# Gaukler/PlainRenderer

Measured on AMD Instinct MI355X. Metric: frames/sec full GI+shade+post @4K; %HBM roofline; 1/2/4/8-GPU scaling, higher is better.
Workload: dtype f32

## Files before the change

plainrenderer_amd/csrc/kernels_fast/shading_fast.hip:

```cpp
#include "../backend.h"
#include "../device/shading_common.h"
#include "../device/fastmath.h"
#include "../device/buffer_fetch.h"
#include "upscale_quad.h"
#include "pcf_taps.h"
#include <cstdlib>
#include <type_traits>

namespace plr {

namespace fastshade {

#ifndef PLR_SHADE_WAVES
#define PLR_SHADE_WAVES 5
#endif

PLR_DI float rcpf(float x) { return __builtin_amdgcn_rcpf(x); }
PLR_DI float rsqf(float x) { return __builtin_amdgcn_rsqf(x); }
PLR_DI float sqrtv(float x) { return __builtin_amdgcn_sqrtf(x); }
PLR_DI float fmin1(float a, float b) { return __builtin_fminf(a, b); }
PLR_DI float fmax1(float a, float b) { return __builtin_fmaxf(a, b); }
PLR_DI float fclamp(float x, float lo, float hi) { return __builtin_fminf(__builtin_fmaxf(x, lo), hi); }
PLR_DI float fmix(float a, float b, float t) { return a + (b - a) * t; }
PLR_DI float log2h(float x) { return __builtin_amdgcn_logf(x); }
// ... 21 lines not shown
    const float inv = rcpRN(sqrtRN((vx * vx + vy * vy) + vz * vz));
    o.Vn = vec3(vx * inv, vy * inv, vz * inv);
    return o;
}
struct Surface { vec3 passPos; float pixelDepth; };
PLR_DI Surface exactSurface(const GlobalUbo* __restrict__ g, vec3 Vn, float depth) {
#pragma clang fp contract(off)
    const float cx = -Vn.x, cy = -Vn.y, cz = -Vn.z;
    const float fx = g->cameraForward[0], fy = g->cameraForward[1], fz = g->cameraForward[2];
    const float dvf = (cx * fx + cy * fy) + cz * fz;
    const float den = g->farPlane + (-depth + 1.f) * (g->nearPlane - g->farPlane);
    const float depthLinear = divRN(g->nearPlane * g->farPlane, den);
    const float rd = rcpf(dvf);
    Surface s;
    s.passPos.x = g->cameraPosition[0] + divRNr(cx, dvf, rd) * depthLinear;
    s.passPos.y = g->cameraPosition[1] + divRNr(cy, dvf, rd) * depthLinear;
    s.passPos.z = g->cameraPosition[2] + divRNr(cz, dvf, rd) * depthLinear;
    const float wx = g->cameraPosition[0] - s.passPos.x, wy = g->cameraPosition[1] - s.passPos.y, wz = g->cameraPosition[2] - s.passPos.z;
    s.pixelDepth = (wx * -fx + wy * -fy) + wz * -fz;
    return s;
}

PLR_DI float D_GGX(float NoH, float r) {
    const float a = NoH * r;
    const float k = r * rcpf(1.0f - NoH * NoH + a * a);
    return k * k * (1.0f / PLR_GLSL_PI);
}
PLR_DI float Visibility(float NoV, float NoL, float r) {
    const float r_2 = r * r;
    const float v1 = NoL * sqrtv(NoV * NoV * (1.f - r_2) + r_2);
    const float v2 = NoV * sqrtv(NoL * NoL * (1.f - r_2) + r_2);
    return 0.5f * rcpf(v1 + v2);
}
PLR_DI vec3 F_Schlick(vec3 f0, vec3 f90, float VoH) { return f0 + (f90 - f0) * pow5(1.f - VoH); }
PLR_DI vec3 DisneyDiffuse(vec3 diffuseColor, float NoL, float VoH, float NoV, float r) {
    const float energyBias = 0.5f * r;
    const float energyFactor = fmix(1.f, 1.f / 1.51f, r);
    const float f90 = energyBias + 2.f * VoH * VoH * r;
    const float fl = 1.f + (f90 - 1.f) * pow5(1.f - NoL), fv = 1.f + (f90 - 1.f) * pow5(1.f - NoV);
    return diffuseColor * ((1.f / PLR_GLSL_PI) * fl * fv * energyFactor);
}
PLR_DI vec3 CoDWWIIDiffuse(vec3 diffuseColor, float NoL, float VoH, float NoV, float NoH, float r) {
    const float f0Diffuse = VoH + pow5(1.f - VoH);
    const float f1 = (1.f - 0.75f * pow5(1.f - NoL)) * (1.f - 0.75f * pow5(1.f - NoV));
    const float g = log2h(2.f * rcpf(r * r) - 1.f) * (1.f / 18.f);
    const float t = fclamp(2.2f * g - 0.5f, 0.f, 1.f);
    const float fd = f0Diffuse + (f1 - f0Diffuse) * t;
    const float fb = (34.5f * g * g - 59.f * g + 24.5f) * VoH * exp2h(-fmax1(73.2f * g - 21.2f, 8.9f) * sqrtv(NoH));
    return diffuseColor * ((1.f / PLR_GLSL_PI) * (fd + fb));
}
PLR_DI float Titanfall2DiffuseSingleComponent(float NoL, float LoV, float NoV, float NoH, float r) {
    const float facing = 0.5f + 0.5f * LoV;
    const float rough = facing * (0.9f - 0.4f * facing) * (0.5f + NoH) * rcpf(fmax1(NoH, 0.03f));
    const float smoothDiffuse = 1.05f * (1.f - pow5(1.f - NoL)) * (1.f - pow5(1.f - NoV));
    return (1.f / PLR_GLSL_PI) * fmix(smoothDiffuse, rough, r);
}
PLR_DI vec3 GGXSingleScattering(float r, vec3 f0, float NoH, float NoV, float VoH, float NoL) {
    return (D_GGX(NoH, r) * Visibility(NoV, NoL, r)) * F_Schlick(f0, vec3(1.f), VoH);
}
PLR_DI float ReflectedEnergyAverage(float roughness) {
    const float smoothness = 1.f - sqrtv(roughness);
    float r = -0.0761947f - 0.383026f * smoothness;
    r = 1.04997f + smoothness * r;
    r = 0.409255f + smoothness * r;
    return fmin1(0.999f, r);
}
PLR_DI float sRGBToLinear1(float c) {
    const float lin = c * (1.f / 12.92f), pw = fpow((c + 0.055f) * (1.f / 1.055f), 2.4f);
    return c <= 0.004045f ? lin : pw;
}

PLR_DI _Float16 halfLo(uint32_t w) { return __builtin_bit_cast(_Float16, (uint16_t)(w & 0xffffu)); }
PLR_DI _Float16 halfHi(uint32_t w) { return __builtin_bit_cast(_Float16, (uint16_t)(w >> 16)); }
PLR_DI vec4 accumulateTexel(vec4 acc, uint32_t xy, uint32_t zw, float w) {
    return vec4(__builtin_fmaf((float)halfLo(xy), w, acc.x), __builtin_fmaf((float)halfHi(xy), w, acc.y), __builtin_fmaf((float)halfLo(zw), w, acc.z),
                __builtin_fmaf((float)halfHi(zw), w, acc.w));
}
PLR_DI void edgePair(int i0, float a, int w, int* xb, float* a2) {
    *xb = clampTo(i0, w - 2);
    *a2 = __builtin_amdgcn_fmed3f(a + (float)(i0 - *xb), 0.f, 1.f);
}

PLR_DI vec4 bilinearLut(const ImgView& im, float u, float v) {
    int i0, j0; float a, b;
    linearCoord(u * (float)im.w, &i0, &a);
    linearCoord(v * (float)im.h, &j0, &b);
    int xb; float a2;
    edgePair(i0, a, im.w, &xb, &a2);
    const int y0 = clampi(j0, im.h), y1 = clampi(j0 + 1, im.h);
    const BufferDesc texels = texelBuffer(im.ptr, 8u);
    const uint4 q0 = fetch128(texels, __umul24((uint32_t)y0, (uint32_t)im.w) + (uint32_t)xb), q1 = fetch128(texels, __umul24((uint32_t)y1, (uint32_t)im.w) + (uint32_t)xb);
    const float a0 = 1.f - a2, b0 = 1.f - b;
    vec4 r(0.f);
    r = accumulateTexel(r, q0.x, q0.y, a0 * b0);
    r = accumulateTexel(r, q0.z, q0.w, a2 * b0);
    r = accumulateTexel(r, q1.x, q1.y, a0 * b);
    r = accumulateTexel(r, q1.z, q1.w, a2 * b);
    return r;
}

struct ShadeParams {
    ImgView color, depth, normal, albedo, specular, brdfLut, shadowMaps[4], ysh, cocg, volumetricLut, skyLut;
    const LightBuffer* light;
    const ShadowCascadeInfo* shadowInfo;
    const VolumetricLightingSettings* vol;
    const GlobalUbo* g;
    const ImgView* bindless;
    uint32_t bindlessCount;
    uint32_t cascadeCount;
    int coverW, coverH, yBase;
    int xBase;
    uint32_t* sig;
    ImgView noiseTex;
    const float4* pcfTaps;
    const float4* pcfTapsByPosition;
    uint32_t pcfPositions;
    const uint2* lutEnergyFootprint;
    const uint32_t* lutEnergyNonFinite;
    uint32_t skipUnlit;
};
PLR_DI float uniformValue(float x) { return u2f((uint32_t)__builtin_amdgcn_readfirstlane((int)f2u(x))); }
PLR_DI bool finiteBits(float x) { return (f2u(x) & 0x7f800000u) != 0x7f800000u; }

#define PLR_SHADE_UNIFORM_PARAMS const GlobalUbo* __restrict__ gUniform, const LightBuffer* __restrict__ lightUniform, const ShadowCascadeInfo* __restrict__ shadowUniform, \
                                 const VolumetricLightingSettings* __restrict__ volUniform
#define PLR_SHADE_ADOPT_UNIFORMS(P) do { (P).g = gUniform; (P).light = lightUniform; (P).shadowInfo = shadowUniform; (P).vol = volUniform; } while (0)
#define PLR_SHADE_UNIFORM_ARGS(P) (P).g, (P).light, (P).shadowInfo, (P).vol

struct PcfTapRow { float4 q[kPcfTaps / 2]; };
PLR_DI float calcShadow(vec3 pos, const ImgView& shadowMap, const float* __restrict__ m, float lssX, float lssY, const PcfTapRow& taps) {
    float cxy0, cxy1;
    uint32_t depthThreshold;
    {
#pragma clang fp contract(off)
        const float x = ((m[0] * pos.x + m[4] * pos.y) + m[8] * pos.z) + m[12];
        const float y = ((m[1] * pos.x + m[5] * pos.y) + m[9] * pos.z) + m[13];
        const float z = ((m[2] * pos.x + m[6] * pos.y) + m[10] * pos.z) + m[14];
        const float w = ((m[3] * pos.x + m[7] * pos.y) + m[11] * pos.z) + m[15];
        const float rw = rcpf(w);
        cxy0 = divRNr(x, w, rw) * 0.5f + 0.5f;
        cxy1 = divRNr(y, w, rw) * 0.5f + 0.5f;
        const float actualDepth = fclamp(divRNr(z, w, rw), 0.f, 1.f);
        const uint32_t t0 = (uint32_t)(actualDepth * 65535.f);
        const float r16 = 1.f / 65535.f;
        const float q1 = divRNr((float)(t0 + 1u), 65535.f, r16), q0 = divRNr((float)t0, 65535.f, r16);
        depthThreshold = q1 <= actualDepth ? t0 + 1u : (q0 <= actualDepth ? t0 : t0 - 1u);
    }
    const int w = shadowMap.w, h = shadowMap.h;
    const float fw = (float)w, fh = (float)h;
    const float bxw = fastm::clampCoord(cxy0 * fw), byh = fastm::clampCoord(cxy1 * fh);
    const float sxw = 0.03f * lssX * fw, syh = 0.03f * lssY * fh;
    const __amdgpu_buffer_rsrc_t map = __builtin_amdgcn_make_buffer_rsrc(shadowMap.ptr, 0, w * h * 2, 0x00020000);
    uint32_t lit = 0u;
// ... 1 lines not shown
        const int xi = floorToInt(__builtin_fmaf(ox, sxw, bxw)), yi = floorToInt(__builtin_fmaf(oy, syh, byh));
        const int t = __mul24(yi, w) + xi;
        const uint32_t off = (uint32_t)xi < (uint32_t)w ? (uint32_t)(t + t) : 0xffffffffu;
        const uint32_t texel = __builtin_amdgcn_raw_buffer_load_b16(map, (int)off, 0, 0);
        lit += texel <= depthThreshold ? 1u : 0u;
    };
#pragma unroll
    for (int k = 0; k < kPcfTaps / 2; k++) {
        const float4 q = taps.q[k];
        tap(q.x, q.y);
        tap(q.z, q.w);
    }
    return (float)lit * (1.f / 12.f);
}

PLR_DI float lutEnergy(const ShadeParams& P, float u, float v) {
    const ImgView& im = P.brdfLut;
    if (!P.lutEnergyFootprint) return bilinearLut(im, u, v).y;
    int i0, j0; float a, b;
    linearCoord(u * (float)im.w, &i0, &a);
    linearCoord(v * (float)im.h, &j0, &b);
    int xb, yb; float a2, b2;
    edgePair(i0, a, im.w, &xb, &a2);
    edgePair(j0, b, im.h, &yb, &b2);
    const uint2 q = P.lutEnergyFootprint[__umul24((uint32_t)yb, (uint32_t)(im.w - 1)) + (uint32_t)xb];
    const float a0 = 1.f - a2, b0 = 1.f - b2;
    float e = (float)halfLo(q.x) * (a0 * b0);
    e = __builtin_fmaf((float)halfHi(q.x), a2 * b0, e);
    e = __builtin_fmaf((float)halfLo(q.y), a0 * b2, e);
    e = __builtin_fmaf((float)halfHi(q.y), a2 * b2, e);
    return e;
}

template <int MULTISCATTER>
PLR_DI vec3 specularMultiscatteringLobe(const ShadeParams& P, float r, float NoL, vec3 f0, vec3 singleScatteringLobe, vec3 brdfLut) {
    const float energyOutgoing = brdfLut.y;
    const vec3 fresnelAverage = f0 + (1.f - f0) * (1.f / 21.f);
    if (MULTISCATTER == 0) {
        const float energyAverage = ReflectedEnergyAverage(r);
        const float energyIncoming = lutEnergy(P, r, NoL);
        const float unscaled = (1.f - energyIncoming) * (1.f - energyOutgoing) * rcpf(3.1415f * (1.f - energyAverage));
        const vec3 den = 1.f - fresnelAverage * (1.f - energyAverage);
        const vec3 scaling = (fresnelAverage * fresnelAverage * energyAverage) * vec3(rcpf(den.x), rcpf(den.y), rcpf(den.z));
        return unscaled * scaling;
    } else if (MULTISCATTER == 1) {
        const float lobe = (1.f - energyOutgoing) * (1.f / PLR_GLSL_PI);
        const vec3 den = 1.f - fresnelAverage * (1.f - energyOutgoing);
        return (fresnelAverage * fresnelAverage * (energyOutgoing * lobe)) * vec3(rcpf(den.x), rcpf(den.y), rcpf(den.z));
    } else if (MULTISCATTER == 2) {
        return f0 * (rcpf(energyOutgoing) - 1.f) * singleScatteringLobe;
    }
    return vec3(0.f);
}

struct PixelInputs {
    float depth;
    uint32_t albedo, specular;
    uint32_t normal, normalH, normalV;
    uint2 ysh;
    uint32_t cocg;
};
PLR_DI vec3 decodeNormal(uint32_t texel) {
    const vec3 raw = fastm::unorm8x4(texel).xyz() * 2.f - 1.f;
    return raw * rsqf(fmax1(dot(raw, raw), 1e-30f));
}

struct SurfaceTerms {
    vec3 N, V, f0, diffuseColor, diffuseBRDFIntegral;
    float r, NoV, energyOutgoing;
    vec3 brdfLut;
};
struct DirectOut { vec3 direct; float pixelDepth; vec2 noiseTexel; };
template <int DIFFUSE_BRDF, int MULTISCATTER, bool GEOMETRIC_AA>
PLR_DI DirectOut shadeDirect(const ShadeParams& P, bool skipUnlit, int px, int py, const ViewRay& vr, const PixelInputs& in, vec3 lightColor, SurfaceTerms* st,
                             uint32_t* sigWord) {
    constexpr bool kLobesSkippable = DIFFUSE_BRDF != 3 && (MULTISCATTER == 0 || MULTISCATTER == 3);
    uint32_t lutNonFinite = 1u;
    if (kLobesSkippable && MULTISCATTER == 0 && skipUnlit && P.lutEnergyNonFinite) lutNonFinite = *P.lutEnergyNonFinite;
    const GlobalUbo* g = P.g;
    const Surface surf = exactSurface(g, vr.Vn, in.depth);
    const vec3 passPos = surf.passPos;
    const float pixelDepth = surf.pixelDepth;

    const vec3 albedoTexel = fastm::unorm8x4(in.albedo).xyz();
    const vec3 specularTexel = fastm::unorm8x4(in.specular).xyz();
    const float metalic = specularTexel.z;
    float r = specularTexel.y;
    r = fmax1(r * r, 0.0045f);
    const vec3 albedo(sRGBToLinear1(albedoTexel.x), sRGBToLinear1(albedoTexel.y), sRGBToLinear1(albedoTexel.z));
    const vec3 diffuseColor = (1.f - metalic) * albedo;
    const vec3 N = decodeNormal(in.normal);
    const vec3 L = nrm(ld3(g->sunDirection));
    const vec3 Lu(uniformValue(L.x), uniformValue(L.y), uniformValue(L.z));
    const vec3 V = vr.Vn;
    if (GEOMETRIC_AA) {
        const vec3 N_U = decodeNormal(in.normalH) - N, N_V = decodeNormal(in.normalV) - N;
        const float variance = 0.25f * (dot(N_V, N_V) + dot(N_U, N_U));
        const float kernelRoughness2 = fmin1(2.f * variance, 0.18f);
        r = fclamp(sqrtv(r * r + kernelRoughness2), 0.f, 1.f);
    }
    const float NdotL = dot(N, L);
    const float NoL = fclamp(NdotL, 0.f, 1.f);
    const bool backFacing = NdotL <= 0.f;
    const float NoV = fmax1(fabsf(dot(N, V)), 0.0001f);
    const vec3 f0 = vmix(vec3(0.04f), albedo, metalic);

    const ImgView noiseTex = P.noiseTex;
    const uint32_t noiseIndex = fastm::texelIndex((uint32_t)fastm::repeatIndex(px, noiseTex.w), (uint32_t)fastm::repeatIndex(py, noiseTex.h), (uint32_t)noiseTex.w);
    const uint32_t noiseWord = fetch16(texelBuffer(noiseTex.ptr, 2u), noiseIndex);
    const vec2 noiseTexel = fastm::unorm8x2(noiseWord);
    const uint32_t noiseByte = noiseWord & 0xffu;

    int cascadeIndex = 0;
#pragma unroll
    for (int cascade = 0; cascade < 3; cascade++) cascadeIndex += (cascade < (int)P.cascadeCount - 1 && pixelDepth >= P.shadowInfo->splits[cascade]) ? 1 : 0;
    const bool skipLobes = kLobesSkippable && skipUnlit && (MULTISCATTER != 0 || __builtin_amdgcn_readfirstlane(lutNonFinite) == 0u);
    float sunShadow = 0.f;
    if (!(skipUnlit && backFacing)) {
        PcfTapRow tapRow;
        {
            const bool byPosition = P.pcfTapsByPosition != nullptr;
            const uint8_t* base = byPosition ? (const uint8_t*)P.pcfTapsByPosition : (const uint8_t*)P.pcfTaps;
            const uint32_t rowStride = byPosition ? P.pcfPositions * 16u : 16u;
            const uint32_t laneOffset = byPosition ? noiseIndex * 16u : noiseByte * (uint32_t)(kPcfTaps / 2 * 16);
            const __amdgpu_buffer_rsrc_t table = __builtin_amdgcn_make_buffer_rsrc((void*)base, 0, 0x7fffffff, 0x00020000);
#pragma unroll
            for (int k = 0; k < kPcfTaps / 2; k++) {
                const auto q = __builtin_amdgcn_raw_buffer_load_b128(table, (int)laneOffset, (int)((uint32_t)k * rowStride), 0);
                __builtin_memcpy(&tapRow.q[k], &q, 16);
            }
        }
        for (bool pending = true; pending;) {
            int c = __builtin_amdgcn_readfirstlane(cascadeIndex);
            const bool mine = cascadeIndex == c;
            asm volatile("" : "+s"(c));
            if (mine) {
                const ImgView& m0 = P.shadowMaps[0];
                ImgView shadowMap;
// ... 2 lines not shown
                shadowMap.h = c == 0 ? m0.h : c == 1 ? P.shadowMaps[1].h : c == 2 ? P.shadowMaps[2].h : P.shadowMaps[3].h;
                shadowMap.d = 1; shadowMap.fmt = F_D16;
                sunShadow = calcShadow(passPos, shadowMap, P.shadowInfo->lightMatrices[c], P.shadowInfo->lightSpaceScale[c][0], P.shadowInfo->lightSpaceScale[c][1], tapRow);
                pending = false;
            }
        }
    }
    *sigWord = (uint32_t)cascadeIndex | ((uint32_t)(sunShadow * 12.f + 0.5f) << 2) | 64u;
    const vec3 brdfLut = bilinearLut(P.brdfLut, r, NoV).xyz();

    const vec3 VL = V + Lu;
    const float VL2 = dot(VL, VL);
    const bool unlit = skipLobes && (backFacing || sunShadow == 0.f) && VL2 >= 1e-30f && VL2 <= 8.f;
    vec3 direct(0.f);
    vec3 diffuseBRDFIntegral(brdfLut.z);
    if (!unlit) {
        const vec3 H = VL * rsqf(VL2);
        const float NoH = fmax1(dot(N, H), 0.f);
        const float VoH = fabsf(dot(V, H));
        const float LoV = fmax1(dot(Lu, V), 0.f);
        const vec3 directLighting = (fmax1(NdotL, 0.f) * sunShadow) * lightColor;
        vec3 diffuseDirect;
        if (DIFFUSE_BRDF == 0) diffuseDirect = diffuseColor * (1.f / PLR_GLSL_PI) * directLighting;
        else if (DIFFUSE_BRDF == 1) diffuseDirect = DisneyDiffuse(diffuseColor, NoL, VoH, NoV, r) * directLighting;
        else if (DIFFUSE_BRDF == 2) diffuseDirect = CoDWWIIDiffuse(diffuseColor, NoL, VoH, NoV, NoH, r) * directLighting;
        else {
            const float single = Titanfall2DiffuseSingleComponent(NoL, LoV, NoV, NoH, r);
            diffuseDirect = diffuseColor * (single + diffuseColor * (0.1159f * r)) * directLighting;
            float multiIntegral = 0.1159f * r * PLR_GLSL_PI * 2.f;
            multiIntegral *= (1.f - (0.04f + 0.96f * pow5(1.f - NoV)));
            multiIntegral *= 0.94291f;
            diffuseBRDFIntegral = vmin(vec3(brdfLut.z) + diffuseColor * multiIntegral, vec3(1.f));
        }
        diffuseDirect = diffuseDirect * ((1.f - F_Schlick(f0, vec3(1.f), NoV)) * (1.f - F_Schlick(f0, vec3(1.f), NoL)));

        const vec3 singleScatteringLobe = GGXSingleScattering(r, f0, NoH, NoV, VoH, NoL);
        const vec3 multiScatteringLobe = specularMultiscatteringLobe<MULTISCATTER>(P, r, NoL, f0, singleScatteringLobe, brdfLut);
        const vec3 specularDirect = directLighting * (singleScatteringLobe + multiScatteringLobe);
        direct = diffuseDirect + specularDirect;
    }

    st->N = N; st->V = V; st->f0 = f0; st->diffuseColor = diffuseColor; st->diffuseBRDFIntegral = diffuseBRDFIntegral;
    st->r = r; st->NoV = NoV; st->energyOutgoing = brdfLut.y; st->brdfLut = brdfLut;
    DirectOut o;
    o.direct = direct;
    o.pixelDepth = pixelDepth;
    o.noiseTexel = noiseTexel;
    return o;
}

template <int MULTISCATTER>
PLR_DI vec3 shadeIndirect(const ShadeParams& P, const SurfaceTerms& st, uint2 ysh, uint32_t cocg) {
    const vec3 N = st.N, V = st.V, f0 = st.f0;
    const float r = st.r, NoV = st.NoV;
    const vec4 irradiance_Y_SH(halfBitsToFloat(ysh.x & 0xffffu), halfBitsToFloat(ysh.x >> 16), halfBitsToFloat(ysh.y & 0xffffu), halfBitsToFloat(ysh.y >> 16));
    const vec2 cc(halfBitsToFloat(cocg & 0xffffu), halfBitsToFloat(cocg >> 16));
    const vec4 shN(0.5f, -0.8660254f * N.y, 0.8660254f * N.z, -0.8660254f * N.x);
    const float irradiance_Y = dot(irradiance_Y_SH, shN);
    const vec3 irradiance = YCoCgToLinear(vec3(irradiance_Y, cc.x, cc.y));
    const vec3 diffuseIndirect = irradiance * st.diffuseColor * st.diffuseBRDFIntegral;
    const vec3 dominantDirection = dominantDirectionFromSH_L1(irradiance_Y_SH);
    const float dominantDirectionLength = fclamp(sqrtv(dot(dominantDirection, dominantDirection)), 0.01f, 1.f);
    const float r_indirect = fmix(1.f, r, sqrtv(dominantDirectionLength));
    const vec3 L_indirect = dominantDirection * rcpf(dominantDirectionLength);
    const vec3 H_indirect = nrm(L_indirect + V);
    const float NoH_indirect = fmax1(dot(N, H_indirect), 0.f);
    const float NoL_indirect = fmax1(dot(N, L_indirect), 0.f);
    const float VoH_indirect = fmax1(dot(V, H_indirect), 0.f);
    const vec3 single_i = GGXSingleScattering(r_indirect, f0, NoH_indirect, NoV, VoH_indirect, NoL_indirect);
    const vec3 multi_i = specularMultiscatteringLobe<MULTISCATTER>(P, r_indirect, NoL_indirect, f0, single_i, vec3(0.f, st.energyOutgoing, 0.f));
    const vec3 specularIndirect = (single_i + multi_i) * YCoCgToLinear(vec3(irradiance_Y_SH.x, cc.x, cc.y));
    return diffuseIndirect + specularIndirect;
}

PLR_DI vec4 froxelLookup(const ShadeParams& P, float su, float sv, vec2 noiseTexel, float pixelDepth) {
    const float nu = su + (noiseTexel.x - 0.5f) * 0.013f, nv = sv + (noiseTexel.y - 0.5f) * 0.013f;
    const float linear = pixelDepth * rcpf(P.vol->maxDistance);
    const float z = log2h(linear * 19.0855369f + 1.f) * (0.693147181f / 3.f);
    const ImgView& vol = P.volumetricLut;
    int i0, j0, k0; float a, b, c;
    linearCoord(nu * (float)vol.w, &i0, &a);
    linearCoord(nv * (float)vol.h, &j0, &b);
    linearCoord(z * (float)vol.d, &k0, &c);
    int xb; float a2;
    edgePair(i0, a, vol.w, &xb, &a2);
    const uint32_t y0 = __umul24((uint32_t)clampi(j0, vol.h), (uint32_t)vol.w), y1 = __umul24((uint32_t)clampi(j0 + 1, vol.h), (uint32_t)vol.w);
    const uint32_t sl = (uint32_t)vol.w * (uint32_t)vol.h;
    const uint32_t z0 = __umul24((uint32_t)clampi(k0, vol.d), sl), z1 = __umul24((uint32_t)clampi(k0 + 1, vol.d), sl);
    const BufferDesc texels = texelBuffer(vol.ptr, 8u);
    const uint32_t x0 = (uint32_t)xb;
    const uint4 q00 = fetch128(texels, z0 + y0 + x0), q01 = fetch128(texels, z0 + y1 + x0), q10 = fetch128(texels, z1 + y0 + x0), q11 = fetch128(texels, z1 + y1 + x0);
    const float a0 = 1.f - a2, b0 = 1.f - b, c0 = 1.f - c;
    const float wab00 = a0 * b0, wab10 = a2 * b0, wab01 = a0 * b, wab11 = a2 * b;
    vec4 it(0.f);
    it = accumulateTexel(it, q00.x, q00.y, wab00 * c0);
    it = accumulateTexel(it, q00.z, q00.w, wab10 * c0);
    it = accumulateTexel(it, q01.x, q01.y, wab01 * c0);
    it = accumulateTexel(it, q01.z, q01.w, wab11 * c0);
    it = accumulateTexel(it, q10.x, q10.y, wab00 * c);
    it = accumulateTexel(it, q10.z, q10.w, wab10 * c);
    it = accumulateTexel(it, q11.x, q11.y, wab01 * c);
    it = accumulateTexel(it, q11.z, q11.w, wab11 * c);
    return it;
}

template <int DIFFUSE_BRDF, int MULTISCATTER, bool GEOMETRIC_AA, int INDIRECT_TECH>
PLR_DI uint32_t shadeGeometryPixel(const ShadeParams& P, int px, int py, const ViewRay& vr, const PixelInputs& in, uint32_t* sigWord) {
    SurfaceTerms st;
    const vec3 sunColor = ld3(P.light->sunColor);
    const bool skipUnlit = P.skipUnlit && finiteBits(sunColor.x) && finiteBits(sunColor.y) && finiteBits(sunColor.z) && finiteBits(P.light->sunStrengthExposed);
    const DirectOut d = shadeDirect<DIFFUSE_BRDF, MULTISCATTER, GEOMETRIC_AA>(P, skipUnlit, px, py, vr, in, sunColor, &st, sigWord);
    vec3 lightingIndirect;
    if (INDIRECT_TECH == 0) lightingIndirect = shadeIndirect<MULTISCATTER>(P, st, in.ysh, in.cocg);
    else {
        const float amb = 0.003f * P.light->sunStrengthExposed;
        const vec3 singleScattering = vmix(vec3(st.brdfLut.x), vec3(st.brdfLut.y), st.f0);
        lightingIndirect = (amb * st.diffuseColor) * st.diffuseBRDFIntegral + singleScattering * amb;
    }
    vec3 outColor = d.direct * P.light->sunStrengthExposed + lightingIndirect;
    const vec4 it = froxelLookup(P, vr.su, vr.sv, d.noiseTexel, d.pixelDepth);
    outColor = outColor * it.w + it.xyz();
    return packR11G11B10(outColor);
}

template <int DIFFUSE_BRDF, int MULTISCATTER, bool GEOMETRIC_AA, int INDIRECT_TECH>
__global__ __launch_bounds__(256, PLR_SHADE_WAVES) void deferredShadingFastKernel(ShadeParams P, PLR_SHADE_UNIFORM_PARAMS) {
    PLR_SHADE_ADOPT_UNIFORMS(P);
    const int px = P.xBase + (int)(blockIdx.x * 64u + (threadIdx.x & 63u));
    const int py = P.yBase + (int)(blockIdx.y * 4u + (threadIdx.x >> 6));
    if (px >= P.coverW || py >= P.coverH) return;
    const ViewRay vr = exactViewRay(P.g, px, py);
    const uint32_t idx = fastm::texelIndex((uint32_t)px, (uint32_t)py, (uint32_t)P.color.w);
    PixelInputs in;
    in.depth = ((const float*)P.depth.ptr)[idx];
    if (in.depth == 0.f) {
        ((uint32_t*)P.color.ptr)[idx] = packR11G11B10(fastm::sampleSkyLut(-vr.Vn, P.skyLut));
        if (P.sig) P.sig[idx] = 128u;
        return;
    }
    in.albedo = ((const uint32_t*)P.albedo.ptr)[idx];
    in.specular = ((const uint32_t*)P.specular.ptr)[idx];
    const uint32_t* normals = (const uint32_t*)P.normal.ptr;
    const uint32_t nw = (uint32_t)P.normal.w;
    const int nx = clampi(px, P.normal.w), ny = clampi(py, P.normal.h);
// ... 33 lines not shown
    const int k0 = (X0 >> 1) - 1, m0 = (Y0 >> 1) - 1;
    const GlobalUbo* g = P.g;
    const float nearP = g->nearPlane, farP = g->farPlane, nf = nearP * farP, nmf = nearP - farP;
    if (t < kGiTileW * kGiTileH) {
        const int r = t / kGiTileW, c = t - r * kGiTileW;
        const int hw = U.srcYSH.w, hh = U.srcYSH.h;
        const uint32_t i = fastm::texelIndex((uint32_t)clampi(k0 + c, hw), (uint32_t)clampi(m0 + r, hh), (uint32_t)hw);
        const uint2 ys = fetch64(texelBuffer(U.srcYSH.ptr, 8u), i);
        const uint32_t cc = fetch32(texelBuffer(U.srcCoCg.ptr, 4u), i);
        GiTexel e;
        e.depthLinear = fastquad::linearDepthRounded(halfBitsToFloat(fetch16(texelBuffer(U.halfResDepth.ptr, 2u), i)), nf, nmf, farP);
        e.y0 = halfBitsToFloat(ys.x & 0xffffu); e.y1 = halfBitsToFloat(ys.x >> 16); e.y2 = halfBitsToFloat(ys.y & 0xffffu); e.y3 = halfBitsToFloat(ys.y >> 16);
        e.co = halfBitsToFloat(cc & 0xffffu); e.cg = halfBitsToFloat(cc >> 16); e.pad = 0.f;
        tile[r][c] = e;
    }
    const int px = X0 + (t & 63), py = Y0 + (t >> 6);
    const bool covered = px < P.coverW && py < P.coverH;
    const int cpx = covered ? px : 0, cpy = covered ? py : 0;
    const uint32_t idx = fastm::texelIndex((uint32_t)cpx, (uint32_t)cpy, (uint32_t)P.color.w);
    PixelInputs in;
    in.depth = u2f(fetch32(texelBuffer(P.depth.ptr, 4u), idx));
    in.albedo = fetch32(texelBuffer(P.albedo.ptr, 4u), idx);
    in.specular = fetch32(texelBuffer(P.specular.ptr, 4u), idx);
    const uint32_t* normals = (const uint32_t*)P.normal.ptr;
    in.normal = fetch32(texelBuffer(P.normal.ptr, 4u), idx);
    in.normalH = in.normalV = in.normal;
    if (GEOMETRIC_AA) {
        in.normalH = fetch32(texelBuffer(P.normal.ptr, 4u), fastm::texelIndex((uint32_t)clampi(cpx ^ 1, P.normal.w), (uint32_t)cpy, (uint32_t)P.normal.w));
        in.normalV = fetch32(texelBuffer(P.normal.ptr, 4u), fastm::texelIndex((uint32_t)cpx, (uint32_t)clampi(cpy ^ 1, P.normal.h), (uint32_t)P.normal.w));
    }
    const ViewRay vr = exactViewRay(g, cpx, cpy);
    __syncthreads();
    if (!covered) return;
    uint32_t upSig;
    {
#pragma clang fp contract(off)
        const int p = px & 1, q = py & 1;
        const int kc = (px >> 1) - k0, mr = (py >> 1) - m0;
        const int c0 = kc - 1 + p, r0 = mr - 1 + q;
        const GiTexel f00 = tile[r0][c0], f10 = tile[r0][c0 + 1], f01 = tile[r0 + 1][c0], f11 = tile[r0 + 1][c0 + 1];
        const float full = fastquad::linearDepthRounded(in.depth, nf, nmf, farP);
        const float ds[4] = {f01.depthLinear, f11.depthLinear, f10.depthLinear, f00.depthLinear};
        const int offx[4] = {0, 1, 1, 0}, offy[4] = {1, 1, 0, 0};
        float minDiff = 1000.f;
        int cx = 0, cy = 0;
        bool isEdge = false;
#pragma unroll
        for (int i = 0; i < 4; i++) {
            const float diff = fabsf(ds[i] - full);
            isEdge = isEdge || diff > 0.5f;
            if (diff < minDiff) { minDiff = diff; cx = offx[i]; cy = offy[i]; }
        }
        float y0, y1, y2, y3, co, cg;
        if (isEdge) {
            const int hw = U.srcYSH.w, hh = U.srcYSH.h;
            const GiTexel n = tile[min((py >> 1) + cy, hh - 1) - m0][min((px >> 1) + cx, hw - 1) - k0];
            y0 = n.y0; y1 = n.y1; y2 = n.y2; y3 = n.y3; co = n.co; cg = n.cg;
        } else {
            const float a = p ? 0.25f : 0.75f, b = q ? 0.25f : 0.75f;
            const float w00 = (1.f - a) * (1.f - b), w10 = a * (1.f - b), w01 = (1.f - a) * b, w11 = a * b;
            auto bl = [&](float t00, float t10, float t01, float t11) { return __builtin_fmaf(t11, w11, __builtin_fmaf(t01, w01, __builtin_fmaf(t10, w10, t00 * w00))); };
            y0 = bl(f00.y0, f10.y0, f01.y0, f11.y0); y1 = bl(f00.y1, f10.y1, f01.y1, f11.y1); y2 = bl(f00.y2, f10.y2, f01.y2, f11.y2); y3 = bl(f00.y3, f10.y3, f01.y3, f11.y3);
            co = bl(f00.co, f10.co, f01.co, f11.co); cg = bl(f00.cg, f10.cg, f01.cg, f11.cg);
        }
        in.ysh = make_uint2(floatToHalfBits(y0) | (floatToHalfBits(y1) << 16), floatToHalfBits(y2) | (floatToHalfBits(y3) << 16));
        in.cocg = floatToHalfBits(co) | (floatToHalfBits(cg) << 16);
        upSig = (isEdge ? 1u : 0u) | (cx ? 2u : 0u) | (cy ? 4u : 0u);
    }
// ... 12 lines not shown
    if (P.sig) P.sig[idx] = sigWord | (upSig << 8);
}

struct DirectRecords { uint4* a; uint4* b; uint32_t* c; };
PLR_DI uint32_t packHalves(float lo, float hi) { return __builtin_bit_cast(uint32_t, __builtin_amdgcn_cvt_pkrtz(lo, hi)); }

template <int DIFFUSE_BRDF, int MULTISCATTER, bool GEOMETRIC_AA>
__global__ __launch_bounds__(256, PLR_SHADE_WAVES) void shadeDirectKernel(ShadeParams P, DirectRecords R, const GlobalUbo G, const ShadowCascadeInfo* __restrict__ shadowUniform,
                                                                          const VolumetricLightingSettings* __restrict__ volUniform) {
    P.g = &G; P.shadowInfo = shadowUniform; P.vol = volUniform; P.light = nullptr;
    const int px = P.xBase + (int)(blockIdx.x * 64u + (threadIdx.x & 63u));
    const int py = P.yBase + (int)(blockIdx.y * 4u + (threadIdx.x >> 6));
    if (px >= P.coverW || py >= P.coverH) return;
    const ViewRay vr = exactViewRay(P.g, px, py);
    const uint32_t idx = fastm::texelIndex((uint32_t)px, (uint32_t)py, (uint32_t)P.color.w);
    PixelInputs in;
    in.depth = u2f(fetch32(texelBuffer(P.depth.ptr, 4u), idx));
    if (in.depth == 0.f) {
        R.a[idx] = make_uint4(packR11G11B10(fastm::sampleSkyLut(-vr.Vn, P.skyLut)), 0u, 0u, 0u);
        return;
    }
    in.albedo = fetch32(texelBuffer(P.albedo.ptr, 4u), idx);
    in.specular = fetch32(texelBuffer(P.specular.ptr, 4u), idx);
    in.normal = fetch32(texelBuffer(P.normal.ptr, 4u), idx);
    in.normalH = in.normalV = in.normal;
    if (GEOMETRIC_AA) {
        in.normalH = fetch32(texelBuffer(P.normal.ptr, 4u), fastm::texelIndex((uint32_t)clampi(px ^ 1, P.normal.w), (uint32_t)py, (uint32_t)P.normal.w));
        in.normalV = fetch32(texelBuffer(P.normal.ptr, 4u), fastm::texelIndex((uint32_t)px, (uint32_t)clampi(py ^ 1, P.normal.h), (uint32_t)P.normal.w));
    }
    in.ysh = make_uint2(0u, 0u);
    in.cocg = 0u;
    SurfaceTerms st;
    uint32_t sigWord;
    const DirectOut d = shadeDirect<DIFFUSE_BRDF, MULTISCATTER, GEOMETRIC_AA>(P, P.skipUnlit != 0u, px, py, vr, in, vec3(1.f), &st, &sigWord);
    const vec4 it = froxelLookup(P, vr.su, vr.sv, d.noiseTexel, d.pixelDepth);
    const vec3 X = d.direct * it.w;
    const vec3 dci = st.diffuseColor * st.diffuseBRDFIntegral;
    R.a[idx] = make_uint4(f2u(X.x), f2u(X.y), f2u(X.z), packHalves(it.w, st.r));
    R.b[idx] = make_uint4(packHalves(it.x, it.y), packHalves(it.z, st.energyOutgoing), packHalves(dci.x, dci.y), packHalves(dci.z, st.f0.x));
    R.c[idx] = packHalves(st.f0.y, st.f0.z);
}

template <int MULTISCATTER>
__global__ __launch_bounds__(256) void upscaleAndCombineKernel(ShadeParams P, FusedUpscale U, DirectRecords R, const GlobalUbo* __restrict__ gUniform, const LightBuffer* __restrict__ lightUniform) {
    P.g = gUniform; P.light = lightUniform;
    __shared__ GiTexel tile[kGiTileH][kGiTileW];
    const int t = (int)threadIdx.x;
    const int X0 = P.xBase + (int)(blockIdx.x * 64u), Y0 = P.yBase + (int)(blockIdx.y * 4u);
    const int k0 = (X0 >> 1) - 1, m0 = (Y0 >> 1) - 1;
    const GlobalUbo* g = P.g;
    const float nearP = g->nearPlane, farP = g->farPlane, nf = nearP * farP, nmf = nearP - farP;
    if (t < kGiTileW * kGiTileH) {
        const int r = t / kGiTileW, c = t - r * kGiTileW;
        const int hw = U.srcYSH.w, hh = U.srcYSH.h;
        const uint32_t i = fastm::texelIndex((uint32_t)clampi(k0 + c, hw), (uint32_t)clampi(m0 + r, hh), (uint32_t)hw);
        const uint2 ys = fetch64(texelBuffer(U.srcYSH.ptr, 8u), i);
        const uint32_t cc = fetch32(texelBuffer(U.srcCoCg.ptr, 4u), i);
        GiTexel e;
        e.depthLinear = fastquad::linearDepthRounded(halfBitsToFloat(fetch16(texelBuffer(U.halfResDepth.ptr, 2u), i)), nf, nmf, farP);
        e.y0 = halfBitsToFloat(ys.x & 0xffffu); e.y1 = halfBitsToFloat(ys.x >> 16); e.y2 = halfBitsToFloat(ys.y & 0xffffu); e.y3 = halfBitsToFloat(ys.y >> 16);
        e.co = halfBitsToFloat(cc & 0xffffu); e.cg = halfBitsToFloat(cc >> 16); e.pad = 0.f;
        tile[r][c] = e;
    }
    const int px = X0 + (t & 63), py = Y0 + (t >> 6);
    const bool covered = px < P.coverW && py < P.coverH;
    const int cpx = covered ? px : 0, cpy = covered ? py : 0;
    const uint32_t idx = fastm::texelIndex((uint32_t)cpx, (uint32_t)cpy, (uint32_t)P.color.w);
// ... 33 lines not shown
            const float w00 = (1.f - a) * (1.f - b), w10 = a * (1.f - b), w01 = (1.f - a) * b, w11 = a * b;
            auto bl = [&](float t00, float t10, float t01, float t11) { return __builtin_fmaf(t11, w11, __builtin_fmaf(t01, w01, __builtin_fmaf(t10, w10, t00 * w00))); };
            y0 = bl(f00.y0, f10.y0, f01.y0, f11.y0); y1 = bl(f00.y1, f10.y1, f01.y1, f11.y1); y2 = bl(f00.y2, f10.y2, f01.y2, f11.y2); y3 = bl(f00.y3, f10.y3, f01.y3, f11.y3);
            co = bl(f00.co, f10.co, f01.co, f11.co); cg = bl(f00.cg, f10.cg, f01.cg, f11.cg);
        }
        ysh = make_uint2(floatToHalfBits(y0) | (floatToHalfBits(y1) << 16), floatToHalfBits(y2) | (floatToHalfBits(y3) << 16));
        cocg = floatToHalfBits(co) | (floatToHalfBits(cg) << 16);
    }
    if (U.storeUpscaled) {
        ((uint2*)U.dstYSH.ptr)[idx] = ysh;
        ((uint32_t*)U.dstCoCg.ptr)[idx] = cocg;
    }
    if (depth == 0.f) {
        ((uint32_t*)P.color.ptr)[idx] = ra.x;
        return;
    }
    SurfaceTerms st;
    st.N = decodeNormal(normalTexel);
    {
        const float su = ((float)px + 0.5f) * rcpf((float)g->screenResolution[0]), sv = ((float)py + 0.5f) * rcpf((float)g->screenResolution[1]);
        const float ndx = su * 2.f - 1.f, ndy = sv * 2.f - 1.f;
        const float ty = g->cameraTanFovHalf * ndy, tx = (g->cameraTanFovHalf * g->cameraAspectRatio) * ndx;
        st.V = nrm(vec3((-g->cameraForward[0] + ty * g->cameraUp[0]) - tx * g->cameraRight[0], (-g->cameraForward[1] + ty * g->cameraUp[1]) - tx * g->cameraRight[1],
                        (-g->cameraForward[2] + ty * g->cameraUp[2]) - tx * g->cameraRight[2]));
    }
    st.NoV = fmax1(fabsf(dot(st.N, st.V)), 0.0001f);
    const float transmittance = (float)halfLo(ra.w);
    st.r = (float)halfHi(ra.w);
    st.energyOutgoing = (float)halfHi(rb.y);
    st.diffuseColor = vec3((float)halfLo(rb.z), (float)halfHi(rb.z), (float)halfLo(rb.w));
    st.diffuseBRDFIntegral = vec3(1.f);
    st.f0 = vec3((float)halfHi(rb.w), (float)halfLo(rc), (float)halfHi(rc));
    st.brdfLut = vec3(0.f);
    const vec3 lightingIndirect = shadeIndirect<MULTISCATTER>(P, st, ysh, cocg);
    const vec3 inScattering((float)halfLo(rb.x), (float)halfHi(rb.x), (float)halfLo(rb.y));
    const vec3 light = ld3(P.light->sunColor) * P.light->sunStrengthExposed;
    const vec3 outColor = vec3(u2f(ra.x), u2f(ra.y), u2f(ra.z)) * light + (lightingIndirect * transmittance + inScattering);
    ((uint32_t*)P.color.ptr)[idx] = packR11G11B10(outColor);
}

typedef void (*ShadeKernel)(ShadeParams, const GlobalUbo*, const LightBuffer*, const ShadowCascadeInfo*, const VolumetricLightingSettings*);
template <int D, int M, bool G> static ShadeKernel pickIndirect(int tech) {
    return tech == 0 ? (ShadeKernel)deferredShadingFastKernel<D, M, G, 0> : (ShadeKernel)deferredShadingFastKernel<D, M, G, 1>;
}
template <int D, int M> static ShadeKernel pickAA(bool aa, int tech) { return aa ? pickIndirect<D, M, true>(tech) : pickIndirect<D, M, false>(tech); }
template <int D> static ShadeKernel pickMulti(int m, bool aa, int tech) {
    switch (m) {
        case 0: return pickAA<D, 0>(aa, tech);
        case 1: return pickAA<D, 1>(aa, tech);
        case 2: return pickAA<D, 2>(aa, tech);
        default: return pickAA<D, 3>(aa, tech);
    }
}
typedef void (*FusedKernel)(ShadeParams, FusedUpscale, const GlobalUbo*, const LightBuffer*, const ShadowCascadeInfo*, const VolumetricLightingSettings*);
template <int D, int M> static FusedKernel pickFusedAA(bool aa) { return aa ? (FusedKernel)upscaleAndShadeKernel<D, M, true> : (FusedKernel)upscaleAndShadeKernel<D, M, false>; }
template <int D> static FusedKernel pickFusedMulti(int m, bool aa) {
    switch (m) {
        case 0: return pickFusedAA<D, 0>(aa);
        case 1: return pickFusedAA<D, 1>(aa);
        case 2: return pickFusedAA<D, 2>(aa);
        default: return pickFusedAA<D, 3>(aa);
    }
}

constexpr int kNoiseSlots = 4;
constexpr uint32_t kMaxNoisePositions = 4096;
// ... 92 lines not shown
    if (int rc = c.needSampled(15, F_RGBA16F, "deferredShading indirectDiffuse_Y_SH")) return rc;
    if (int rc = c.needSampled(16, F_RG16F, "deferredShading indirectDiffuse_CoCg")) return rc;
    if (int rc = c.needSampled(18, F_RGBA16F, "deferredShading volumetricLightingLUT")) return rc;
    if (int rc = c.needUbuf(19, 52, "deferredShading volumetric settings")) return rc;
    if (int rc = c.needSampled(20, F_D32, "deferredShading depth")) return rc;
    if (int rc = c.needSampled(21, F_RGBA8, "deferredShading world normals")) return rc;
    if (int rc = c.needSampled(22, F_RGBA8, "deferredShading albedo")) return rc;
    if (int rc = c.needSampled(23, F_RGBA8, "deferredShading specular")) return rc;
    if (int rc = c.needSampled(24, F_R11G11B10, "deferredShading skyLut")) return rc;
    if (!c.bindless || c.bindlessCount == 0) return c.fail(-4, "deferredShading: global texture array (set 2) is empty");
    if (c.sampled[16].w != c.sampled[15].w || c.sampled[16].h != c.sampled[15].h) return c.fail(-4, "deferredShading: Y_SH and CoCg differ in size");
    for (int b : {20, 22, 23}) if (c.sampled[b].w != c.storage[0].w || c.sampled[b].h != c.storage[0].h) return kUseGeneralKernel;
    if (c.sampled[3].w < 2 || c.sampled[18].w < 2) return kUseGeneralKernel;
    *diffuseBRDF = c.specInt(0, 0); *multi = c.specInt(1, 0); *tech = c.specInt(3, 0);
    *aa = c.specBool(2, false);
    const uint32_t cascades = c.specUint(4, 4u);
    if (*diffuseBRDF < 0 || *diffuseBRDF > 3 || *multi < 0 || *multi > 3 || cascades < 1 || cascades > 4) return c.fail(-1, "deferredShading: specialisation constant out of range");
    ShadeParams P{};
    P.color = c.storage[0]; P.depth = c.sampled[20]; P.normal = c.sampled[21]; P.albedo = c.sampled[22]; P.specular = c.sampled[23];
    P.brdfLut = c.sampled[3];
    for (int i = 0; i < 4; i++) P.shadowMaps[i] = c.sampled[9 + i];
    P.ysh = c.sampled[15]; P.cocg = c.sampled[16]; P.volumetricLut = c.sampled[18]; P.skyLut = c.sampled[24];
    P.light = (const LightBuffer*)c.sbuf[7].ptr; P.shadowInfo = (const ShadowCascadeInfo*)c.sbuf[8].ptr;
    P.vol = (const VolumetricLightingSettings*)c.ubuf[19].ptr; P.g = c.global;
    P.bindless = c.bindless; P.bindlessCount = c.bindlessCount; P.cascadeCount = cascades;
    if (!c.hostNoiseView(&P.noiseTex)) return kUseGeneralKernel;
    if (deriveTables) if (int rc = shadeDerivedTables(c, &P, records)) return rc;
    const PassCtx::RowSpan rs = c.rowSpan(P.color.h);
    const PassCtx::ColSpan cs = c.colSpan(P.color.w);
    P.coverW = cs.x1; P.xBase = cs.x0; P.coverH = rs.y1; P.yBase = rs.y0;
    P.sig = c.sigFor((size_t)P.color.w * (size_t)P.color.h);
    const char* skipEnv = std::getenv("PLR_SHADE_SKIP_UNLIT");
    P.skipUnlit = (!P.sig && !(skipEnv && skipEnv[0] == '0' && skipEnv[1] == 0)) ? 1u : 0u;
    *out = P;
    return 0;
}

static int launchDeferredShadingFast(const PassCtx& c) {
    ShadeParams P;
    int diffuseBRDF, multi, tech;
    bool aa;
    if (int rc = shadeParamsFor(c, &P, &diffuseBRDF, &multi, &aa, &tech)) return rc;
    ShadeKernel k = nullptr;
    switch (diffuseBRDF) {
        case 0: k = pickMulti<0>(multi, aa, tech); break;
        case 1: k = pickMulti<1>(multi, aa, tech); break;
        case 2: k = pickMulti<2>(multi, aa, tech); break;
        default: k = pickMulti<3>(multi, aa, tech); break;
    }
    if (P.coverW <= P.xBase || P.coverH <= P.yBase) return 0;
    k<<<dim3(divUp((unsigned)(P.coverW - P.xBase), 64u), divUp((unsigned)(P.coverH - P.yBase), 4u)), 256, 0, c.stream>>>(P, PLR_SHADE_UNIFORM_ARGS(P));
    PLR_CHECK_LAUNCH(c);
    return 0;
}

struct FusedShade { ShadeParams P; FusedUpscale U; int diffuseBRDF, multi; bool aa; };
static int fusedShadeSetup(const PassCtx* const* ctxs, size_t count, FusedShade* f, bool deriveTables, DirectRecords* records) {
    if (count != 2) return kUseGeneralKernel;
    const PassCtx &u = *ctxs[0], &c = *ctxs[1];
    if (!u.global || !u.hasStorage(0) || !u.hasStorage(1) || !u.hasSampled(2) || !u.hasSampled(3) || !u.hasSampled(4) || !u.hasSampled(5)) return kUseGeneralKernel;
    if (u.storage[0].fmt != F_RGBA16F || u.storage[1].fmt != F_RG16F || u.sampled[2].fmt != F_RGBA16F || u.sampled[3].fmt != F_RG16F || u.sampled[4].fmt != F_D32 ||
        u.sampled[5].fmt != F_R16F)
        return kUseGeneralKernel;
    const ImgView& out = u.storage[0];
    const PassCtx::RowSpan ur = u.rowSpan(out.h);
    const bool regular = out.w == 2 * u.sampled[2].w && out.h == 2 * u.sampled[2].h && u.sampled[3].w == u.sampled[2].w && u.sampled[3].h == u.sampled[2].h &&
// ... 12 lines not shown
    if (c.global != u.global || !u.globalHost || u.globalHost->screenResolution[0] != out.w || u.globalHost->screenResolution[1] != out.h) return kUseGeneralKernel;
    FusedUpscale& U = f->U;
    U.srcYSH = u.sampled[2]; U.srcCoCg = u.sampled[3]; U.halfResDepth = u.sampled[5]; U.dstYSH = u.storage[0]; U.dstCoCg = u.storage[1];
    U.storeUpscaled = 1;
    return 0;
}

typedef void (*DirectKernel)(ShadeParams, DirectRecords, const GlobalUbo, const ShadowCascadeInfo*, const VolumetricLightingSettings*);
template <int D, int M> static DirectKernel pickDirectAA(bool aa) { return aa ? (DirectKernel)shadeDirectKernel<D, M, true> : (DirectKernel)shadeDirectKernel<D, M, false>; }
template <int D> static DirectKernel pickDirectMulti(int m, bool aa) {
    switch (m) {
        case 0: return pickDirectAA<D, 0>(aa);
        case 1: return pickDirectAA<D, 1>(aa);
        case 2: return pickDirectAA<D, 2>(aa);
        default: return pickDirectAA<D, 3>(aa);
    }
}

static int earlyShadeDirect(const PassCtx* const* ctxs, size_t count, EarlyPart& part) {
    FusedShade f;
    DirectRecords R{};
    const bool launch = part.mode == EarlyPart::Launch;
    if (int rc = fusedShadeSetup(ctxs, count, &f, launch, launch ? &R : nullptr)) return rc;
    const PassCtx& c = *ctxs[1];
    if (!c.globalHost || c.sigFor(1)) return kUseGeneralKernel;
    if (!launch) {
        const ShadeParams& P = f.P;
        for (const void* k : {(const void*)P.depth.ptr, (const void*)P.normal.ptr, (const void*)P.albedo.ptr, (const void*)P.specular.ptr, (const void*)P.brdfLut.ptr,
                              (const void*)P.shadowMaps[0].ptr, (const void*)P.shadowMaps[1].ptr, (const void*)P.shadowMaps[2].ptr, (const void*)P.shadowMaps[3].ptr,
                              (const void*)P.volumetricLut.ptr, (const void*)P.skyLut.ptr, (const void*)P.shadowInfo, (const void*)P.vol, (const void*)P.noiseTex.ptr})
            part.reads->push_back(k);
        return 0;
    }
    const ShadeParams& P = f.P;
    if (P.coverH <= P.yBase || P.coverW <= P.xBase) return 0;
    DirectKernel k = nullptr;
    switch (f.diffuseBRDF) {
        case 0: k = pickDirectMulti<0>(f.multi, f.aa); break;
        case 1: k = pickDirectMulti<1>(f.multi, f.aa); break;
        case 2: k = pickDirectMulti<2>(f.multi, f.aa); break;
        default: k = pickDirectMulti<3>(f.multi, f.aa); break;
    }
    k<<<dim3(divUp((unsigned)(P.coverW - P.xBase), 64u), divUp((unsigned)(P.coverH - P.yBase), 4u)), 256, 0, c.stream>>>(P, R, *c.globalHost, P.shadowInfo, P.vol);
    PLR_CHECK_LAUNCH(c);
    return 0;
}

static int launchUpscaleAndShade(const PassCtx* const* ctxs, size_t count) {
    FusedShade f;
    DirectRecords R{};
    const bool late = count == 2 && ctxs[0]->earlyPartDone;
    if (int rc = fusedShadeSetup(ctxs, count, &f, true, late ? &R : nullptr)) return rc;
    const PassCtx &u = *ctxs[0], &c = *ctxs[1];
    const ShadeParams& P = f.P;
    FusedUpscale& U = f.U;
    if (P.coverH <= P.yBase || P.coverW <= P.xBase) return 0;
    U.storeUpscaled = (u.elidableStorage & 3u) == 3u ? 0 : 1;
    if (!U.storeUpscaled) u.elidedStorage = 3u;
    const dim3 grid(divUp((unsigned)(P.coverW - P.xBase), 64u), divUp((unsigned)(P.coverH - P.yBase), 4u));
    if (late) {
        switch (f.multi) {
            case 0: upscaleAndCombineKernel<0><<<grid, 256, 0, c.stream>>>(P, U, R, P.g, P.light); break;
            case 1: upscaleAndCombineKernel<1><<<grid, 256, 0, c.stream>>>(P, U, R, P.g, P.light); break;
            case 2: upscaleAndCombineKernel<2><<<grid, 256, 0, c.stream>>>(P, U, R, P.g, P.light); break;
            default: upscaleAndCombineKernel<3><<<grid, 256, 0, c.stream>>>(P, U, R, P.g, P.light); break;
        }
        PLR_CHECK_LAUNCH(c);
        return 0;
    }
    FusedKernel k = nullptr;
    switch (f.diffuseBRDF) {
        case 0: k = pickFusedMulti<0>(f.multi, f.aa); break;
        case 1: k = pickFusedMulti<1>(f.multi, f.aa); break;
        case 2: k = pickFusedMulti<2>(f.multi, f.aa); break;
        default: k = pickFusedMulti<3>(f.multi, f.aa); break;
    }
    k<<<grid, 256, 0, c.stream>>>(P, U, PLR_SHADE_UNIFORM_ARGS(P));
    PLR_CHECK_LAUNCH(c);
    return 0;
}

constexpr int kLutSamples = 1024;
template <int DIFFUSE_BRDF>
__global__ __launch_bounds__(256) void brdfLutFastKernel(ImgView lut, int coverW, int coverH) {
    __shared__ float4 ggx[kLutSamples];
    __shared__ float4 cosine[kLutSamples];
    for (int i = (int)threadIdx.x; i < kLutSamples; i += 256) {
        const float x0 = (float)i * (1.f / (float)kLutSamples);
        uint32_t bits = (uint32_t)i;
        bits = __builtin_bitreverse32(bits);
        const float x1 = (float)bits * 2.3283064365386963e-10f;
        float sg, cg, sp, cp;
        det_sincosf(2.f * PLR_GLSL_PI * x0, &sg, &cg);
// ... 89 lines not shown
```

Baseline: 1468.

## Add wave-uniform fast paths: scalar Fresnel for dielectric waves, skip upscale for sky waves

Adds a per-launch wavePaths flag, set through an environment variable and on by default when no signature buffer is used, that turns on two wave-level fast paths. When a ballot shows that no lane in a 64-wide wave has nonzero metalness bits, the sun and indirect specular lobes are evaluated with a scalar Fresnel instead of a vec3, which removes about two thirds of that ALU work. When every lane in a wave is sky (depth zero) and upscaled storage is elided, the quad upscale of GI samples is skipped entirely. The cost is extra template instantiations, more divergent code and register pressure, and it relies on f0 being grey when metalness is zero.

```diff
diff --git a/plainrenderer_amd/csrc/kernels_fast/shading_fast.hip b/plainrenderer_amd/csrc/kernels_fast/shading_fast.hip
--- a/plainrenderer_amd/csrc/kernels_fast/shading_fast.hip
+++ b/plainrenderer_amd/csrc/kernels_fast/shading_fast.hip
@@ -77,7 +77,9 @@
     const float v2 = NoV * sqrtv(NoL * NoL * (1.f - r_2) + r_2);
     return 0.5f * rcpf(v1 + v2);
 }
-PLR_DI vec3 F_Schlick(vec3 f0, vec3 f90, float VoH) { return f0 + (f90 - f0) * pow5(1.f - VoH); }
+PLR_DI float rcpEach(float x) { return rcpf(x); }
+PLR_DI vec3 rcpEach(vec3 v) { return vec3(rcpf(v.x), rcpf(v.y), rcpf(v.z)); }
+template <class F> PLR_DI F F_Schlick(F f0, F f90, float VoH) { return f0 + (f90 - f0) * pow5(1.f - VoH); }
 PLR_DI vec3 DisneyDiffuse(vec3 diffuseColor, float NoL, float VoH, float NoV, float r) {
     const float energyBias = 0.5f * r;
     const float energyFactor = fmix(1.f, 1.f / 1.51f, r);
@@ -100,8 +102,8 @@
     const float smoothDiffuse = 1.05f * (1.f - pow5(1.f - NoL)) * (1.f - pow5(1.f - NoV));
     return (1.f / PLR_GLSL_PI) * fmix(smoothDiffuse, rough, r);
 }
-PLR_DI vec3 GGXSingleScattering(float r, vec3 f0, float NoH, float NoV, float VoH, float NoL) {
-    return (D_GGX(NoH, r) * Visibility(NoV, NoL, r)) * F_Schlick(f0, vec3(1.f), VoH);
+template <class F> PLR_DI F GGXSingleScattering(float r, F f0, float NoH, float NoV, float VoH, float NoL) {
+    return (D_GGX(NoH, r) * Visibility(NoV, NoL, r)) * F_Schlick(f0, F(1.f), VoH);
 }
 PLR_DI float ReflectedEnergyAverage(float roughness) {
     const float smoothness = 1.f - sqrtv(roughness);
@@ -163,7 +165,9 @@
     const uint2* lutEnergyFootprint;
     const uint32_t* lutEnergyNonFinite;
     uint32_t skipUnlit;
+    uint32_t wavePaths;
 };
+constexpr uint32_t kWaveSkySkipsUpscale = 1u, kWaveScalarFresnel = 2u, kWaveAllPaths = 3u;
 PLR_DI float uniformValue(float x) { return u2f((uint32_t)__builtin_amdgcn_readfirstlane((int)f2u(x))); }
 PLR_DI bool finiteBits(float x) { return (f2u(x) & 0x7f800000u) != 0x7f800000u; }
 
@@ -231,25 +235,25 @@
     return e;
 }
 
-template <int MULTISCATTER>
-PLR_DI vec3 specularMultiscatteringLobe(const ShadeParams& P, float r, float NoL, vec3 f0, vec3 singleScatteringLobe, vec3 brdfLut) {
+template <int MULTISCATTER, class F>
+PLR_DI F specularMultiscatteringLobe(const ShadeParams& P, float r, float NoL, F f0, F singleScatteringLobe, vec3 brdfLut) {
     const float energyOutgoing = brdfLut.y;
-    const vec3 fresnelAverage = f0 + (1.f - f0) * (1.f / 21.f);
+    const F fresnelAverage = f0 + (1.f - f0) * (1.f / 21.f);
     if (MULTISCATTER == 0) {
         const float energyAverage = ReflectedEnergyAverage(r);
         const float energyIncoming = lutEnergy(P, r, NoL);
         const float unscaled = (1.f - energyIncoming) * (1.f - energyOutgoing) * rcpf(3.1415f * (1.f - energyAverage));
-        const vec3 den = 1.f - fresnelAverage * (1.f - energyAverage);
-        const vec3 scaling = (fresnelAverage * fresnelAverage * energyAverage) * vec3(rcpf(den.x), rcpf(den.y), rcpf(den.z));
+        const F den = 1.f - fresnelAverage * (1.f - energyAverage);
+        const F scaling = (fresnelAverage * fresnelAverage * energyAverage) * rcpEach(den);
         return unscaled * scaling;
     } else if (MULTISCATTER == 1) {
         const float lobe = (1.f - energyOutgoing) * (1.f / PLR_GLSL_PI);
-        const vec3 den = 1.f - fresnelAverage * (1.f - energyOutgoing);
-        return (fresnelAverage * fresnelAverage * (energyOutgoing * lobe)) * vec3(rcpf(den.x), rcpf(den.y), rcpf(den.z));
+        const F den = 1.f - fresnelAverage * (1.f - energyOutgoing);
+        return (fresnelAverage * fresnelAverage * (energyOutgoing * lobe)) * rcpEach(den);
     } else if (MULTISCATTER == 2) {
         return f0 * (rcpf(energyOutgoing) - 1.f) * singleScatteringLobe;
     }
-    return vec3(0.f);
+    return F(0.f);
 }
 
 struct PixelInputs {
@@ -268,9 +272,10 @@
     vec3 N, V, f0, diffuseColor, diffuseBRDFIntegral;
     float r, NoV, energyOutgoing;
     vec3 brdfLut;
+    bool scalarFresnel;
 };
 struct DirectOut { vec3 direct; float pixelDepth; vec2 noiseTexel; };
-template <int DIFFUSE_BRDF, int MULTISCATTER, bool GEOMETRIC_AA>
+template <int DIFFUSE_BRDF, int MULTISCATTER, bool GEOMETRIC_AA, bool SCALAR_FRESNEL>
 PLR_DI DirectOut shadeDirect(const ShadeParams& P, bool skipUnlit, int px, int py, const ViewRay& vr, const PixelInputs& in, vec3 lightColor, SurfaceTerms* st,
                              uint32_t* sigWord) {
     constexpr bool kLobesSkippable = DIFFUSE_BRDF != 3 && (MULTISCATTER == 0 || MULTISCATTER == 3);
@@ -303,6 +308,7 @@
     const bool backFacing = NdotL <= 0.f;
     const float NoV = fmax1(fabsf(dot(N, V)), 0.0001f);
     const vec3 f0 = vmix(vec3(0.04f), albedo, metalic);
+    const bool scalarFresnel = SCALAR_FRESNEL && (P.wavePaths & kWaveScalarFresnel) && __builtin_amdgcn_ballot_w64((in.specular & 0xff0000u) != 0u) == 0ull;
 
     const ImgView noiseTex = P.noiseTex;
     const uint32_t noiseIndex = fastm::texelIndex((uint32_t)fastm::repeatIndex(px, noiseTex.w), (uint32_t)fastm::repeatIndex(py, noiseTex.h), (uint32_t)noiseTex.w);
@@ -371,16 +377,20 @@
             multiIntegral *= 0.94291f;
             diffuseBRDFIntegral = vmin(vec3(brdfLut.z) + diffuseColor * multiIntegral, vec3(1.f));
         }
-        diffuseDirect = diffuseDirect * ((1.f - F_Schlick(f0, vec3(1.f), NoV)) * (1.f - F_Schlick(f0, vec3(1.f), NoL)));
-
-        const vec3 singleScatteringLobe = GGXSingleScattering(r, f0, NoH, NoV, VoH, NoL);
-        const vec3 multiScatteringLobe = specularMultiscatteringLobe<MULTISCATTER>(P, r, NoL, f0, singleScatteringLobe, brdfLut);
-        const vec3 specularDirect = directLighting * (singleScatteringLobe + multiScatteringLobe);
-        direct = diffuseDirect + specularDirect;
+        auto sunLobes = [&](auto fresnel0) {
+            using F = decltype(fresnel0);
+            const vec3 diffuse = diffuseDirect * ((1.f - F_Schlick(fresnel0, F(1.f), NoV)) * (1.f - F_Schlick(fresnel0, F(1.f), NoL)));
+            const F singleScatteringLobe = GGXSingleScattering(r, fresnel0, NoH, NoV, VoH, NoL);
+            const F multiScatteringLobe = specularMultiscatteringLobe<MULTISCATTER>(P, r, NoL, fresnel0, singleScatteringLobe, brdfLut);
+            const vec3 specularDirect = directLighting * (singleScatteringLobe + multiScatteringLobe);
+            return diffuse + specularDirect;
+        };
+        if (scalarFresnel) direct = sunLobes(f0.x);
+        else direct = sunLobes(f0);
     }
 
     st->N = N; st->V = V; st->f0 = f0; st->diffuseColor = diffuseColor; st->diffuseBRDFIntegral = diffuseBRDFIntegral;
-    st->r = r; st->NoV = NoV; st->energyOutgoing = brdfLut.y; st->brdfLut = brdfLut;
+    st->r = r; st->NoV = NoV; st->energyOutgoing = brdfLut.y; st->brdfLut = brdfLut; st->scalarFresnel = scalarFresnel;
     DirectOut o;
     o.direct = direct;
     o.pixelDepth = pixelDepth;
@@ -406,9 +416,14 @@
     const float NoH_indirect = fmax1(dot(N, H_indirect), 0.f);
     const float NoL_indirect = fmax1(dot(N, L_indirect), 0.f);
     const float VoH_indirect = fmax1(dot(V, H_indirect), 0.f);
-    const vec3 single_i = GGXSingleScattering(r_indirect, f0, NoH_indirect, NoV, VoH_indirect, NoL_indirect);
-    const vec3 multi_i = specularMultiscatteringLobe<MULTISCATTER>(P, r_indirect, NoL_indirect, f0, single_i, vec3(0.f, st.energyOutgoing, 0.f));
-    const vec3 specularIndirect = (single_i + multi_i) * YCoCgToLinear(vec3(irradiance_Y_SH.x, cc.x, cc.y));
+    const vec3 ambient = YCoCgToLinear(vec3(irradiance_Y_SH.x, cc.x, cc.y));
+    auto specularResponse = [&](auto fresnel0) {
+        using F = decltype(fresnel0);
+        const F single_i = GGXSingleScattering(r_indirect, fresnel0, NoH_indirect, NoV, VoH_indirect, NoL_indirect);
+        const F multi_i = specularMultiscatteringLobe<MULTISCATTER>(P, r_indirect, NoL_indirect, fresnel0, single_i, vec3(0.f, st.energyOutgoing, 0.f));
+        return (single_i + multi_i) * ambient;
+    };
+    const vec3 specularIndirect = st.scalarFresnel ? specularResponse(f0.x) : specularResponse(f0);
     return diffuseIndirect + specularIndirect;
 }
 
@@ -448,7 +463,7 @@
     SurfaceTerms st;
     const vec3 sunColor = ld3(P.light->sunColor);
     const bool skipUnlit = P.skipUnlit && finiteBits(sunColor.x) && finiteBits(sunColor.y) && finiteBits(sunColor.z) && finiteBits(P.light->sunStrengthExposed);
-    const DirectOut d = shadeDirect<DIFFUSE_BRDF, MULTISCATTER, GEOMETRIC_AA>(P, skipUnlit, px, py, vr, in, sunColor, &st, sigWord);
+    const DirectOut d = shadeDirect<DIFFUSE_BRDF, MULTISCATTER, GEOMETRIC_AA, INDIRECT_TECH == 0>(P, skipUnlit, px, py, vr, in, sunColor, &st, sigWord);
     vec3 lightingIndirect;
     if (INDIRECT_TECH == 0) lightingIndirect = shadeIndirect<MULTISCATTER>(P, st, in.ysh, in.cocg);
     else {
@@ -548,8 +563,11 @@
     const ViewRay vr = exactViewRay(g, cpx, cpy);
     __syncthreads();
     if (!covered) return;
-    uint32_t upSig;
-    {
+    const bool skyWave = (P.wavePaths & kWaveSkySkipsUpscale) && !U.storeUpscaled && !P.sig && __builtin_amdgcn_ballot_w64(in.depth != 0.f) == 0ull;
+    uint32_t upSig = 0u;
+    in.ysh = make_uint2(0u, 0u);
+    in.cocg = 0u;
+    if (!skyWave) {
 #pragma clang fp contract(off)
         const int p = px & 1, q = py & 1;
         const int kc = (px >> 1) - k0, mr = (py >> 1) - m0;
@@ -628,7 +646,7 @@
     in.cocg = 0u;
     SurfaceTerms st;
     uint32_t sigWord;
-    const DirectOut d = shadeDirect<DIFFUSE_BRDF, MULTISCATTER, GEOMETRIC_AA>(P, P.skipUnlit != 0u, px, py, vr, in, vec3(1.f), &st, &sigWord);
+    const DirectOut d = shadeDirect<DIFFUSE_BRDF, MULTISCATTER, GEOMETRIC_AA, false>(P, P.skipUnlit != 0u, px, py, vr, in, vec3(1.f), &st, &sigWord);
     const vec4 it = froxelLookup(P, vr.su, vr.sv, d.noiseTexel, d.pixelDepth);
     const vec3 X = d.direct * it.w;
     const vec3 dci = st.diffuseColor * st.diffuseBRDFIntegral;
@@ -728,6 +746,7 @@
     st.diffuseBRDFIntegral = vec3(1.f);
     st.f0 = vec3((float)halfHi(rb.w), (float)halfLo(rc), (float)halfHi(rc));
     st.brdfLut = vec3(0.f);
+    st.scalarFresnel = false;
     const vec3 lightingIndirect = shadeIndirect<MULTISCATTER>(P, st, ysh, cocg);
     const vec3 inScattering((float)halfLo(rb.x), (float)halfHi(rb.x), (float)halfLo(rb.y));
     const vec3 light = ld3(P.light->sunColor) * P.light->sunStrengthExposed;
@@ -886,6 +905,8 @@
     P.sig = c.sigFor((size_t)P.color.w * (size_t)P.color.h);
     const char* skipEnv = std::getenv("PLR_SHADE_SKIP_UNLIT");
     P.skipUnlit = (!P.sig && !(skipEnv && skipEnv[0] == '0' && skipEnv[1] == 0)) ? 1u : 0u;
+    const char* pathsEnv = std::getenv("PLR_SHADE_WAVE_PATHS");
+    P.wavePaths = P.sig ? 0u : (pathsEnv && pathsEnv[0] ? (uint32_t)std::strtoul(pathsEnv, nullptr, 0) & kWaveAllPaths : kWaveAllPaths);
     *out = P;
     return 0;
 }
@@ -964,6 +985,7 @@
             part.reads->push_back(k);
         return 0;
     }
+    f.P.wavePaths = 0u;
     const ShadeParams& P = f.P;
     if (P.coverH <= P.yBase || P.coverW <= P.xBase) return 0;
     DirectKernel k = nullptr;
@@ -991,6 +1013,7 @@
     if (!U.storeUpscaled) u.elidedStorage = 3u;
     const dim3 grid(divUp((unsigned)(P.coverW - P.xBase), 64u), divUp((unsigned)(P.coverH - P.yBase), 4u));
     if (late) {
+        f.P.wavePaths = 0u;
         switch (f.multi) {
             case 0: upscaleAndCombineKernel<0><<<grid, 256, 0, c.stream>>>(P, U, R, P.g, P.light); break;
             case 1: upscaleAndCombineKernel<1><<<grid, 256, 0, c.stream>>>(P, U, R, P.g, P.light); break;
```

After: 1482 (median of 6 runs). No clear change (+0.9%).
